# avlmaps/AVLMaps

Hardware: AMD Instinct MI355X
Metric: voxel_query_similarities_per_sec (higher is better)
Workload: dtype f32

## Files before the change

### avlmaps_amd/csrc/avl_sim.hip

```cpp
#include <cfloat>
#include <algorithm>
#include <climits>
#include <cstdlib>
#include <vector>

#include "avl_common.h"

namespace avl {

using half8 = __attribute__((ext_vector_type(8))) _Float16;
using half2 = __attribute__((ext_vector_type(2))) _Float16;
using f32x16 = __attribute__((ext_vector_type(16))) float;
using f32x4 = __attribute__((ext_vector_type(4))) float;

constexpr int kExactQB = 8;

template <bool VEC4>
__global__ __launch_bounds__(256) void sim_exact_kernel(const float* __restrict__ feat, int64_t N, int D, int64_t ld,
                                                        const float* __restrict__ q, int Q, int64_t ldq, int q0,
                                                        float* __restrict__ scores, int32_t* __restrict__ argmax,
                                                        float* __restrict__ best, int first_chunk) {
    extern __shared__ __attribute__((aligned(16))) float qs[];
    const int Dp = (D + 3) & ~3;
    const int qn = min(kExactQB, Q - q0);
// ... 46 lines not shown
            }
        }
#pragma unroll
        for (int r = 0; r < R; ++r)
#pragma unroll
            for (int j = 0; j < kExactQB; ++j) {
#pragma unroll
                for (int off = 32; off > 0; off >>= 1) acc[r][j] += __shfl_xor(acc[r][j], off, 64);
            }
#pragma unroll
        for (int r = 0; r < R; ++r) {
            const int64_t row = row0 + r;
            if (lane == r && row < N) {
                float bv = -INFINITY;
                int bi = q0;
                if (!first_chunk) {
                    if (best) bv = best[row];
                    if (argmax) bi = argmax[row];
                }
                bool have = !first_chunk;
#pragma unroll
                for (int j = 0; j < kExactQB; ++j) {
                    if (j < qn) {
                        if (scores) scores[row * (int64_t)Q + q0 + j] = acc[r][j];
                        if (!have || acc[r][j] > bv) {
                            bv = acc[r][j];
                            bi = q0 + j;
                            have = true;
                        }
                    }
                }
                if (argmax) argmax[row] = bi;
                if (best) best[row] = bv;
            }
        }
    }
}

constexpr int kHdrAlign = 256;
constexpr int kRowPadHalves = 8;
constexpr int kSplitThreads = 512;
#ifdef AVL_RING
template <bool PRE, bool XR, bool QM> struct RingDepth { static constexpr int value = AVL_RING; };
#else
#ifndef AVL_RING_QM
#define AVL_RING_QM 2
#endif
template <bool PRE, bool XR, bool QM> struct RingDepth { static constexpr int value = (!PRE && !XR) ? (QM ? AVL_RING_QM : 3) : 2; };
#endif
constexpr int kTileRows = (kSplitThreads / 64) * 32;

__global__ __launch_bounds__(256) void sim_prep_queries_kernel(const float* __restrict__ q, int Q, int D, int64_t ldq,
                                                               float* __restrict__ inv_scale, _Float16* __restrict__ img,
                                                               int Qtot, int KC, int nkc, int interleaved) {
    __shared__ float red[4];
    __shared__ float scale_s;
    const int qg = blockIdx.x;
    const bool live = qg < Q;
    const float* row = q + (int64_t)qg * ldq;
    float m = 0.f;
    if (live)
        for (int d = threadIdx.x; d < D; d += blockDim.x) m = fmaxf(m, fabsf(row[d]));
    for (int off = 32; off > 0; off >>= 1) m = fmaxf(m, __shfl_xor(m, off, 64));
    if ((threadIdx.x & 63) == 0) red[threadIdx.x >> 6] = m;
    __syncthreads();
    if (threadIdx.x == 0) {
        const float mx = fmaxf(fmaxf(red[0], red[1]), fmaxf(red[2], red[3]));
        int S = 0;
        if (mx > 0.f && isfinite(mx)) S = 9 - ilogbf(mx);
        S = max(-60, min(60, S));
        scale_s = ldexpf(1.f, S);
        inv_scale[qg] = ldexpf(1.f, -S);
    }
    __syncthreads();
    const float scale = scale_s;
    const int rowlen = KC + kRowPadHalves;
    if (interleaved) {
        const int rowblk = 2 * KC + kRowPadHalves;
        for (int kc = 0; kc < nkc; ++kc) {
            _Float16* hi = img + ((int64_t)kc * Qtot + qg) * rowblk;
            for (int kk = threadIdx.x; kk < KC + kRowPadHalves; kk += blockDim.x) {
                const int k = kc * KC + kk;
                float v = 0.f;
                if (live && kk < KC && k < D) v = row[k] * scale;
                const half2 h = __builtin_bit_cast(half2, __builtin_amdgcn_cvt_pkrtz(v, 0.f));
                if (kk < KC) {
                    hi[kk] = h[0];
                    hi[KC + kk] = (_Float16)(v - (float)h[0]);
                } else {
                    hi[KC + kk] = (_Float16)0;
                }
            }
        }
        return;
    }
    for (int kc = 0; kc < nkc; ++kc) {
        _Float16* hi = img + ((int64_t)(kc * 2) * Qtot + qg) * rowlen;
        _Float16* lo = hi + (int64_t)Qtot * rowlen;
        for (int kk = threadIdx.x; kk < rowlen; kk += blockDim.x) {
            const int k = kc * KC + kk;
            float v = 0.f;
            if (live && kk < KC && k < D) v = row[k] * scale;
            const half2 h = __builtin_bit_cast(half2, __builtin_amdgcn_cvt_pkrtz(v, 0.f));
            hi[kk] = h[0];
            lo[kk] = (_Float16)(v - (float)h[0]);
        }
    }
}

__device__ __forceinline__ void split8(const f32x4 v0, const f32x4 v1, half8& hi, half8& lo) {
#ifdef AVL_ABL_NOSPLIT
    hi = __builtin_bit_cast(half8, v0);
    lo = __builtin_bit_cast(half8, v1);
#else
    const float x[8] = {v0.x, v0.y, v0.z, v0.w, v1.x, v1.y, v1.z, v1.w};
    float m1 = -1.0f;
    asm("" : "+v"(m1));
#pragma unroll
    for (int p = 0; p < 4; ++p) {
        half2 h = __builtin_bit_cast(half2, __builtin_amdgcn_cvt_pkrtz(x[2 * p], x[2 * p + 1]));
        float r0 = __builtin_fmaf((float)h[0], m1, x[2 * p]);
        float r1 = __builtin_fmaf((float)h[1], m1, x[2 * p + 1]);
        half2 l = __builtin_bit_cast(half2, __builtin_amdgcn_cvt_pkrtz(r0, r1));
        hi[2 * p] = h[0];
        hi[2 * p + 1] = h[1];
        lo[2 * p] = l[0];
        lo[2 * p + 1] = l[1];
    }
#endif
}

constexpr float kGuardLo = 0x1p-7f, kGuardHi = 0x1p15f;

__device__ __forceinline__ void guard_max8(float& m, const f32x4 v0, const f32x4 v1) {
#ifndef AVL_GUARD_BUILTIN
    asm("v_max3_f32 %0, |%1|, |%2|, %0" : "+v"(m) : "v"(v0.x), "v"(v0.y));
    asm("v_max3_f32 %0, |%1|, |%2|, %0" : "+v"(m) : "v"(v0.z), "v"(v0.w));
    asm("v_max3_f32 %0, |%1|, |%2|, %0" : "+v"(m) : "v"(v1.x), "v"(v1.y));
    asm("v_max3_f32 %0, |%1|, |%2|, %0" : "+v"(m) : "v"(v1.z), "v"(v1.w));
#else
    m = __builtin_fmaxf(__builtin_fmaxf(m, __builtin_fabsf(v0.x)), __builtin_fabsf(v0.y));
    m = __builtin_fmaxf(__builtin_fmaxf(m, __builtin_fabsf(v0.z)), __builtin_fabsf(v0.w));
    m = __builtin_fmaxf(__builtin_fmaxf(m, __builtin_fabsf(v1.x)), __builtin_fabsf(v1.y));
    m = __builtin_fmaxf(__builtin_fmaxf(m, __builtin_fabsf(v1.z)), __builtin_fabsf(v1.w));
#endif
}

template <int QT, int NA, bool XR = false>
__device__ __forceinline__ void split_epilogue(const f32x16 (&acc)[QT][NA], const float* isc, int q_base, int rows, int Q,
                                               float* __restrict__ scores, int32_t* __restrict__ argmax,
                                               float* __restrict__ best, int64_t row, int64_t N, int kg, int first_chunk,
                                               float rscale = 1.f, uint32_t* __restrict__ flags = nullptr, float rmax = 1.f,
                                               const int32_t* qml = nullptr, f32x4 xacc = f32x4{0.f, 0.f, 0.f, 0.f}) {
    int lim = (XR ? 32 * QT : rows) - 4 * kg;
    asm volatile("" : "+v"(lim));
    float bv = -INFINITY;
    int bl = INT_MAX;
#pragma unroll
    for (int t = 0; t < QT; ++t) {
#pragma unroll
        for (int g = 0; g < 4; ++g) {
            const int c0 = t * 32 + 8 * g;
            const int ql = c0 + 4 * kg;
            const int qg = q_base + ql;
            const f32x4 is4 = *reinterpret_cast<const f32x4*>(isc + ql);
            f32x4 v;
            f32x4 r = {acc[t][0][4 * g + 0], acc[t][0][4 * g + 1], acc[t][0][4 * g + 2], acc[t][0][4 * g + 3]};
#pragma unroll
            for (int a = 1; a < NA; ++a) {
                r.x += acc[t][a][4 * g + 0]; r.y += acc[t][a][4 * g + 1]; r.z += acc[t][a][4 * g + 2]; r.w += acc[t][a][4 * g + 3];
            }
            v.x = r.x * is4.x * rscale;
            v.y = r.y * is4.y * rscale;
            v.z = r.z * is4.z * rscale;
            v.w = r.w * is4.w * rscale;
            if (scores && row < N) {
                float* sp = scores + row * (int64_t)Q + qg;
                if (qml) {
                    float* sr = scores + row * (int64_t)Q;
                    const int4 qm4 = *reinterpret_cast<const int4*>(qml + ql);
                    if (c0 + 0 < lim) sr[qm4.x] = v.x;
                    if (c0 + 1 < lim) sr[qm4.y] = v.y;
                    if (c0 + 2 < lim) sr[qm4.z] = v.z;
                    if (c0 + 3 < lim) sr[qm4.w] = v.w;
                } else if (c0 + 3 < lim && (Q & 3) == 0) {
                    *reinterpret_cast<f32x4*>(sp) = v;
                } else {
                    if (c0 + 0 < lim) sp[0] = v.x;
                    if (c0 + 1 < lim) sp[1] = v.y;
                    if (c0 + 2 < lim) sp[2] = v.z;
                    if (c0 + 3 < lim) sp[3] = v.w;
                }
            }
            if (c0 + 0 < lim && v.x > bv) { bv = v.x; bl = c0 + 0; }
            if (c0 + 1 < lim && v.y > bv) { bv = v.y; bl = c0 + 1; }
            if (c0 + 2 < lim && v.z > bv) { bv = v.z; bl = c0 + 2; }
            if (c0 + 3 < lim && v.w > bv) { bv = v.w; bl = c0 + 3; }
        }
    }
    int bi = bl == INT_MAX ? INT_MAX : q_base + 4 * kg + bl;
    float xv[4] = {0.f, 0.f, 0.f, 0.f};
    if constexpr (XR) {
        const f32x4 xis = *reinterpret_cast<const f32x4*>(isc + 32 * QT);
#pragma unroll
        for (int r = 0; r < 4; ++r) xv[r] = (xacc[r] + __shfl_xor(xacc[r], 32, 64)) * xis[r] * rscale;
        if (scores && row < N && kg == 0) {
            float* sr = scores + row * (int64_t)Q;
#pragma unroll
            for (int r = 0; r < 4; ++r)
                if (32 * QT + r < rows) sr[qml ? qml[32 * QT + r] : q_base + 32 * QT + r] = xv[r];
        }
    }
    if (argmax || best || flags) {
        if (qml && bi != INT_MAX) bi = qml[bi - q_base];
        const float ov = __shfl_xor(bv, 32, 64);
        const int oi = __shfl_xor(bi, 32, 64);
        if (ov > bv || (ov == bv && oi < bi)) {
            bv = ov;
            bi = oi;
        }
        if constexpr (XR) {
#pragma unroll
            for (int r = 0; r < 4; ++r)
                if (32 * QT + r < rows && xv[r] > bv) {
                    bv = xv[r];
                    bi = qml ? qml[32 * QT + r] : q_base + 32 * QT + r;
                }
        }
        if (flags) {
            const float m = fmaxf(rmax, __shfl_xor(rmax, 32, 64));
            const bool bad = row < N && (!(m == 0.f || (m >= kGuardLo && m < kGuardHi)) || bi == INT_MAX);
            const unsigned long long mask = __ballot(bad);
            const int64_t row0 = __shfl(row, 0, 64);
            if ((threadIdx.x & 63) == 0 && row0 < N) {
                const uint32_t w = (uint32_t)(mask | (mask >> 32));
                flags[row0 >> 5] = first_chunk ? w : (flags[row0 >> 5] | w);
            }
        }
        if ((argmax || best) && kg == 0 && row < N) {
            if (bi == INT_MAX) bi = qml ? qml[0] : q_base;
            if (!first_chunk) {
                const float pv = best[row];
                const int pi = argmax ? argmax[row] : -1;
                if (pv > bv || (pv == bv && pi < bi)) {
                    bv = pv;
                    bi = argmax ? pi : bi;
                }
            }
            if (argmax) argmax[row] = bi;
            if (best) best[row] = bv;
        }
    }
}

__global__ __launch_bounds__(256) void sim_prepare_map_kernel(float* __restrict__ feat, int64_t N, int D, int64_t ld,
                                                              float* __restrict__ row_scale) {
    const int lane = threadIdx.x & 63;
    const int64_t wave0 = ((int64_t)blockIdx.x * blockDim.x + threadIdx.x) >> 6;
    const int64_t nwaves = ((int64_t)gridDim.x * blockDim.x) >> 6;
    const int gpr = D >> 3;
    for (int64_t row = wave0; row < N; row += nwaves) {
        f32x4* p = reinterpret_cast<f32x4*>(feat + row * ld);
        float scale = 1.f;
        if (row_scale) {
            unsigned mb = 0;
            for (int g = lane; g < 2 * gpr; g += 64) {
                const f32x4 v = p[g];
                mb = max(max(mb, __float_as_uint(v.x) & 0x7fffffffu), __float_as_uint(v.y) & 0x7fffffffu);
                mb = max(max(mb, __float_as_uint(v.z) & 0x7fffffffu), __float_as_uint(v.w) & 0x7fffffffu);
            }
            for (int off = 32; off > 0; off >>= 1) mb = max(mb, (unsigned)__shfl_xor((int)mb, off, 64));
            int sh = 0;
            if (mb != 0 && mb < 0x7f800000u) sh = max(-100, min(100, 14 - ilogbf(__uint_as_float(mb))));
            scale = ldexpf(1.f, sh);
            if (lane == 0) row_scale[row] = mb >= 0x7f800000u ? __uint_as_float(0x7fc00000u) : ldexpf(1.f, -sh);
        }
        for (int g = lane; g < gpr; g += 64) {
            f32x4 v0 = p[2 * g], v1 = p[2 * g + 1];
            v0.x *= scale; v0.y *= scale; v0.z *= scale; v0.w *= scale;
            v1.x *= scale; v1.y *= scale; v1.z *= scale; v1.w *= scale;
            half8 hi, lo;
            split8(v0, v1, hi, lo);
            p[2 * g] = __builtin_bit_cast(f32x4, hi);
            p[2 * g + 1] = __builtin_bit_cast(f32x4, lo);
        }
    }
}

__host__ __device__ __forceinline__ int compact_lo_offset(int c) { return 128 * (c >> 7) + 64 * ((c >> 5) & 1) + 32 * ((c >> 6) & 1) + (c & 31); }

__global__ __launch_bounds__(256) void sim_prepare_map24_kernel(const float* __restrict__ feat, int64_t N, int D, int64_t ld,
                                                                unsigned char* __restrict__ out, float* __restrict__ row_scale) {
    const int lane = threadIdx.x & 63;
    const int64_t wave0 = ((int64_t)blockIdx.x * blockDim.x + threadIdx.x) >> 6;
    const int64_t nwaves = ((int64_t)gridDim.x * blockDim.x) >> 6;
    const int g8 = D >> 3;
    for (int64_t row = wave0; row < N; row += nwaves) {
        const f32x4* p = reinterpret_cast<const f32x4*>(feat + row * ld);
        unsigned mb = 0;
        for (int g = lane; g < 2 * g8; g += 64) {
            const f32x4 v = p[g];
            mb = max(max(mb, __float_as_uint(v.x) & 0x7fffffffu), __float_as_uint(v.y) & 0x7fffffffu);
            mb = max(max(mb, __float_as_uint(v.z) & 0x7fffffffu), __float_as_uint(v.w) & 0x7fffffffu);
        }
        for (int off = 32; off > 0; off >>= 1) mb = max(mb, (unsigned)__shfl_xor((int)mb, off, 64));
        int sh = 0;
        if (mb != 0 && mb < 0x7f800000u) sh = max(-100, min(100, 14 - ilogbf(__uint_as_float(mb))));
        const float scale = ldexpf(1.f, sh);
        if (lane == 0) row_scale[row] = mb >= 0x7f800000u ? __uint_as_float(0x7fc00000u) : ldexpf(1.f, -sh);
        unsigned char* orow = out + row * ((int64_t)D * 3);
        for (int g = lane; g < g8; g += 64) {
            const f32x4 v0 = p[2 * g], v1 = p[2 * g + 1];
            const float x[8] = {v0.x * scale, v0.y * scale, v0.z * scale, v0.w * scale, v1.x * scale, v1.y * scale, v1.z * scale, v1.w * scale};
            half8 hi;
            unsigned u[8];
#pragma unroll
            for (int e = 0; e < 8; ++e) {
                const _Float16 h = (_Float16)x[e];
                hi[e] = h;
                const int eb = (__builtin_bit_cast(unsigned short, h) >> 10) & 31;
                int k = 0;
#ifndef AVL_COMPACT_FIXED_UNITS
                if (eb > 18 && eb < 31) k = (int)rintf((x[e] - (float)h) * ldexpf(1.f, 33 - eb));
#else
                if (eb < 31) k = (int)rintf((x[e] - (float)h) * 16.f);
#endif
                u[e] = (unsigned)(max(-128, min(127, k)) + 128);
            }
            const int w0 = (int)(u[0] | (u[1] << 8) | (u[2] << 16) | (u[3] << 24));
            const int w1 = (int)(u[4] | (u[5] << 8) | (u[6] << 16) | (u[7] << 24));
            *reinterpret_cast<half8*>(orow + (size_t)g * 16) = hi;
            *reinterpret_cast<int2*>(orow + 2 * (size_t)D + compact_lo_offset(8 * g)) = int2{w0, w1};
        }
    }
}

__global__ __launch_bounds__(256) void sim_fixup_rows_kernel(const float* __restrict__ feat, int64_t N, int D, int64_t ld,
                                                             const float* __restrict__ q, int Q, int64_t ldq,
                                                             const uint32_t* __restrict__ flags, float* __restrict__ scores,
                                                             int32_t* __restrict__ argmax, float* __restrict__ best) {
    const int lane = threadIdx.x & 63;
    const int64_t wave0 = ((int64_t)blockIdx.x * blockDim.x + threadIdx.x) >> 6;
    const int64_t nwaves = ((int64_t)gridDim.x * blockDim.x) >> 6;
    const int64_t nwords = (N + 31) >> 5;
    for (int64_t base = wave0 * 64; base < nwords; base += nwaves * 64) {
        const uint32_t w = base + lane < nwords ? flags[base + lane] : 0u;
        unsigned long long any = __ballot(w != 0u);
        while (any) {
            const int l = __ffsll((long long)any) - 1;
            any &= any - 1;
            uint32_t word = (uint32_t)__shfl((int)w, l, 64);
            while (word) {
                const int b = __ffs((int)word) - 1;
                word &= word - 1;
                const int64_t row = (base + l) * 32 + b;
                if (row >= N) continue;
                const float* a = feat + row * ld;
                float bv = -INFINITY;
                int bi = 0;
                bool have = false, nan_seen = false;
                for (int qi = 0; qi < Q; ++qi) {
                    const float* qr = q + (int64_t)qi * ldq;
                    float sum = 0.f;
                    for (int d = lane; d < D; d += 64) sum = fmaf(a[d], qr[d], sum);
                    for (int off = 32; off > 0; off >>= 1) sum += __shfl_xor(sum, off, 64);
                    if (lane == 0 && scores) scores[row * (int64_t)Q + qi] = sum;
                    if (!nan_seen) {
                        if (sum != sum) { nan_seen = true; bv = sum; bi = qi; }
                        else if (!have || sum > bv) { bv = sum; bi = qi; have = true; }
                    }
                }
                if (lane == 0) {
                    if (argmax) argmax[row] = bi;
                    if (best) best[row] = bv;
                }
            }
        }
    }
}

__global__ __launch_bounds__(256) void sim_gather_queries_kernel(const float* __restrict__ q, int64_t ldq, const int32_t* __restrict__ rows,
                                                                 int nrows, int col0, int cols, float* __restrict__ out) {
    const int r = blockIdx.x;
    if (r >= nrows) return;
    const int32_t sr = rows[r];
    const float* src = q + (int64_t)(sr < 0 ? 0 : sr) * ldq + col0;
    float* dst = out + (int64_t)r * cols;
    for (int c = threadIdx.x; c < cols; c += blockDim.x) dst[c] = sr < 0 ? 0.f : src[c];
}


__device__ __forceinline__ void compact_load_step(f32x4 (&b)[8], const char* row, int64_t ld, int kg, int sa) {
    const f32x4* gh = reinterpret_cast<const f32x4*>(row + 128 * sa + 64 * kg);
    const f32x4* gl = reinterpret_cast<const f32x4*>(row + 2 * ld + 128 * (sa >> 1) + 64 * kg + 32 * (sa & 1));
#pragma unroll
    for (int t = 0; t < 4; ++t) b[t] = gh[t];
#pragma unroll
    for (int t = 0; t < 2; ++t) b[4 + t] = gl[t];
}

template <int PAIR>
__device__ __forceinline__ half2 residual_pair(unsigned w, unsigned hi2) {
#ifndef AVL_COMPACT_FIXED_UNITS
    using ushort2v = __attribute__((ext_vector_type(2))) unsigned short;
    const unsigned pat = __builtin_amdgcn_perm(0x64646464u, w, PAIR == 0 ? 0x04010400u : 0x04030402u);
    const half2 k = __builtin_bit_cast(half2, pat) + half2{(_Float16)-1152.0f, (_Float16)-1152.0f};
    const ushort2v e = __builtin_bit_cast(ushort2v, hi2 & 0x7C007C00u);
    const ushort2v sc = __builtin_elementwise_sub_sat(e, ushort2v{0x4800, 0x4800});
    return k * __builtin_bit_cast(half2, sc);
#else
    (void)hi2;
    const unsigned pat = __builtin_amdgcn_perm(0x54545454u, w, PAIR == 0 ? 0x04010400u : 0x04030402u);
    return __builtin_bit_cast(half2, pat) + half2{(_Float16)-72.0f, (_Float16)-72.0f};
#endif
}

__device__ __forceinline__ void compact_operands(const f32x4& hi, const f32x4& lo, int second, half8& bh, half8& bl) {
    bh = __builtin_bit_cast(half8, hi);
    using u32x4 = __attribute__((ext_vector_type(4))) unsigned;
    const u32x4 hw = __builtin_bit_cast(u32x4, hi);
    const u32x4 lw = __builtin_bit_cast(u32x4, lo);
    const unsigned w0 = lw[second * 2], w1 = lw[second * 2 + 1];
    const half2 l0 = residual_pair<0>(w0, hw[0]), l1 = residual_pair<1>(w0, hw[1]);
    const half2 l2 = residual_pair<0>(w1, hw[2]), l3 = residual_pair<1>(w1, hw[3]);
    bl = half8{l0[0], l0[1], l1[0], l1[1], l2[0], l2[1], l3[0], l3[1]};
}

template <bool PRE, bool P24>
__device__ __forceinline__ void map_operands(const f32x4 (&b)[8], int m, half8& bh, half8& bl, float& rmax) {
    if constexpr (P24) {
        compact_operands(b[m], b[4 + (m >> 1)], m & 1, bh, bl);
    } else if constexpr (PRE) {
        bh = __builtin_bit_cast(half8, b[2 * m]);
        bl = __builtin_bit_cast(half8, b[2 * m + 1]);
    } else {
#ifndef AVL_ABL_NOGUARD
        guard_max8(rmax, b[2 * m], b[2 * m + 1]);
#endif
        split8(b[2 * m], b[2 * m + 1], bh, bl);
    }
}

template <int QT, int NSTEPS, bool PRE, bool FQ, bool QM = false, bool P24 = false, bool XR = false>
__global__ __launch_bounds__(kSplitThreads) void sim_split_f16_kernel(
    const float* __restrict__ feat, int64_t N, int D, int64_t ld, const _Float16* __restrict__ img,
    const float* __restrict__ inv_scale, const float* __restrict__ q_raw, int64_t ldq, int Qtot, int KC, int nkc, int q_base,
    int rows, int Q, float* __restrict__ scores, int32_t* __restrict__ argmax, float* __restrict__ best, int first_chunk,
    const float* __restrict__ row_scale, uint32_t* __restrict__ flags, const int32_t* __restrict__ qmap, int col0) {
    extern __shared__ __attribute__((aligned(16))) char smem[];
    constexpr int NA = QT == 1 ? 3 : (QT == 2 ? 2 : 1);
    constexpr int X1 = NA > 1 ? 1 : 0, X2 = NA > 2 ? 2 : X1;
    const int lane = threadIdx.x & 63, wave = threadIdx.x >> 6;
    const int j = lane & 31, kg = lane >> 5;
    const int row_b = (KC + kRowPadHalves) * 2;
    static_assert(!XR || FQ, "the extra-row path builds its query image in the kernel");
    constexpr int TQ = (QT + (XR ? 1 : 0)) * 32;
    const int zrow = (FQ && rows < (XR ? 32 * QT + 4 : 32 * QT)) ? 1 : 0;
    const int img_b = (rows + zrow) * row_b;
    float* isc = reinterpret_cast<float*>(smem + 2 * img_b);
    int32_t* qml = reinterpret_cast<int32_t*>(isc + TQ);
    if constexpr (QM) {
        if (threadIdx.x < TQ) qml[threadIdx.x] = threadIdx.x < rows ? qmap[q_base + threadIdx.x] : INT_MAX;
    }
    if constexpr (!FQ) {
        if (threadIdx.x < TQ) isc[threadIdx.x] = threadIdx.x < rows ? inv_scale[q_base + threadIdx.x] : 0.f;
    } else {
        if (threadIdx.x >= rows && threadIdx.x < TQ) isc[threadIdx.x] = 0.f;
        constexpr int RB = 4, NW = kSplitThreads / 64;
        for (int r0 = wave; r0 < rows; r0 += NW * RB) {
            float v[RB][8];
#pragma unroll
            for (int b = 0; b < RB; ++b) {
                const int r = r0 + NW * b;
                const float* qr = q_raw + (int64_t)(q_base + (r < rows ? r : rows - 1)) * ldq;
#pragma unroll
                for (int t = 0; t < 8; ++t) v[b][t] = (lane + 64 * t < D) ? qr[lane + 64 * t] : 0.f;
            }
#pragma unroll
            for (int b = 0; b < RB; ++b) {
                const int r = r0 + NW * b;
                if (r < rows) {
                    float m = 0.f;
#pragma unroll
                    for (int t = 0; t < 8; ++t) m = fmaxf(m, fabsf(v[b][t]));
                    for (int off = 32; off > 0; off >>= 1) m = fmaxf(m, __shfl_xor(m, off, 64));
                    int S = 0;
                    if (m > 0.f && isfinite(m)) S = 9 - ilogbf(m);
                    S = max(-60, min(60, S));
                    const float scale = ldexpf(1.f, S);
                    if (lane == 0) isc[r] = ldexpf(1.f, -S);
                    _Float16* hi = reinterpret_cast<_Float16*>(smem + r * row_b);
                    _Float16* lo = reinterpret_cast<_Float16*>(smem + img_b + r * row_b);
#pragma unroll
                    for (int t = 0; t < 8; ++t) {
                        const int k = lane + 64 * t;
                        if (k < KC) {
                            const float x = v[b][t] * scale;
                            const half2 h = __builtin_bit_cast(half2, __builtin_amdgcn_cvt_pkrtz(x, 0.f));
                            hi[k] = h[0];
                            lo[k] = (_Float16)(x - (float)h[0]);
                        }
                    }
                    if (lane < kRowPadHalves) {
                        hi[KC + lane] = (_Float16)0;
                        lo[KC + lane] = (_Float16)0;
                    }
                }
            }
        }
        if (zrow) {
            uint32_t* zh = reinterpret_cast<uint32_t*>(smem + rows * row_b);
            uint32_t* zl = reinterpret_cast<uint32_t*>(smem + img_b + rows * row_b);
            for (int i = threadIdx.x; i < row_b / 4; i += kSplitThreads) {
                zh[i] = 0u;
                zl[i] = 0u;
            }
        }
    }

    auto fill_lds = [&](int kc) {
        const char* hi = reinterpret_cast<const char*>(img) + ((int64_t)(kc * 2) * Qtot + q_base) * row_b;
        const char* lo = hi + (int64_t)Qtot * row_b;
        const uint4* s0 = reinterpret_cast<const uint4*>(hi);
        const uint4* s1 = reinterpret_cast<const uint4*>(lo);
        uint4* d0 = reinterpret_cast<uint4*>(smem);
        uint4* d1 = reinterpret_cast<uint4*>(smem + img_b);
        for (int i = threadIdx.x; i < img_b / 16; i += kSplitThreads) {
// ... 123 lines not shown
                f32x4 hb[2][4], lb[2][4];
                auto load_hi = [&](int st) {
                    const f32x4* g = reinterpret_cast<const f32x4*>(rp24 + 128 * (sa0 + st) + 64 * kg);
#pragma unroll
                    for (int t = 0; t < 4; ++t) hb[st & 1][t] = g[t];
                };
                auto load_lo = [&](int blk) {
                    const f32x4* g = reinterpret_cast<const f32x4*>(rp24 + 2 * ld + 128 * ((sa0 >> 1) + blk) + 64 * kg);
#pragma unroll
                    for (int t = 0; t < 4; ++t) lb[blk & 1][t] = g[t];
                };
                load_hi(0);
                load_lo(0);
#pragma unroll
                for (int st = 0; st < NSTEPS; ++st) {
                    if (st + 1 < NSTEPS) {
                        load_hi(st + 1);
                        if (((st + 1) & 1) == 0) load_lo((st + 1) >> 1);
                    }
                    __builtin_amdgcn_sched_barrier(0);
                    compute_with([&](int m, half8& bh, half8& bl) {
                        compact_operands(hb[st & 1][m], lb[(st >> 1) & 1][2 * (st & 1) + (m >> 1)], m & 1, bh, bl);
                    }, st);
                }
            } else if constexpr (NSTEPS > 0) {
                constexpr int kRing = RingDepth<PRE, XR, QM>::value;
                f32x4 ring[kRing][8];
#pragma unroll
                for (int r = 0; r + 1 < kRing; ++r)
                    if (r < NSTEPS) load(ring[r], r);
#pragma unroll
                for (int s = 0; s < NSTEPS; ++s) {
                    if (s + kRing - 1 < NSTEPS) load(ring[(s + kRing - 1) % kRing], s + kRing - 1);
                    __builtin_amdgcn_sched_barrier(0);
                    compute(ring[s % kRing], s);
                }
            } else {
                load(buf0, 0);
                for (int s = 0; s < nsteps; s += 2) {
                    if (s + 1 < nsteps) load(buf1, s + 1);
                    compute(buf0, s);
                    if (s + 1 < nsteps) {
                        if (s + 2 < nsteps) load(buf0, s + 2);
                        compute(buf1, s + 1);
                    }
                }
            }
        }

        float rscale = 1.f;
        if constexpr (PRE) {
            if (row_scale) rscale = row_scale[rowc];
        }
        split_epilogue<QT, NA, XR>(acc, isc, q_base, rows, Q, scores, argmax, best, row, N, kg, first_chunk, rscale, PRE ? nullptr : flags, rmax,
                                   QM ? qml : nullptr, xacc0 + xacc1);
    }
}

template <int QT, int T, int NS, bool PRE, bool QM = false, bool P24 = false>
__global__ __launch_bounds__(kSplitThreads) void sim_kswap_f16_kernel(
    const float* __restrict__ feat, int64_t N, int D, int64_t ld, const _Float16* __restrict__ img,
    const float* __restrict__ inv_scale, int Qtot, int KC, int q_base, int rows, int Q, float* __restrict__ scores,
    int32_t* __restrict__ argmax, float* __restrict__ best, int first_chunk, const float* __restrict__ row_scale,
    uint32_t* __restrict__ flags, const int32_t* __restrict__ qmap, int col0) {
    extern __shared__ __attribute__((aligned(16))) char smem[];
    const int lane = threadIdx.x & 63, wave = threadIdx.x >> 6;
    const int j = lane & 31, kg = lane >> 5;
    const int row_b = (KC + kRowPadHalves) * 2;
    const int zrow = rows < 32 * QT ? 1 : 0;
    const int img_b = (rows + zrow) * row_b;
    float* isc = reinterpret_cast<float*>(smem + 2 * img_b);
    int32_t* qml = reinterpret_cast<int32_t*>(isc + QT * 32);
    if constexpr (QM) {
        if (threadIdx.x < QT * 32) qml[threadIdx.x] = threadIdx.x < rows ? qmap[q_base + threadIdx.x] : INT_MAX;
    }
    if (threadIdx.x < QT * 32) isc[threadIdx.x] = threadIdx.x < rows ? inv_scale[q_base + threadIdx.x] : 0.f;
    auto fill_lds = [&](int kc) {
        using gptr = const __attribute__((address_space(1))) void*;
        using lptr = __attribute__((address_space(3))) void*;
        const char* hi = reinterpret_cast<const char*>(img) + ((int64_t)(kc * 2) * Qtot + q_base) * row_b;
        const char* lo = hi + (int64_t)Qtot * row_b;
        const int nb = rows * row_b;
        for (int c = wave * 1024; c < nb; c += (kSplitThreads / 64) * 1024) {
            if (c + lane * 16 < nb) {
                __builtin_amdgcn_global_load_lds((gptr)(hi + c + lane * 16), (lptr)(smem + c), 16, 0, 0);
                __builtin_amdgcn_global_load_lds((gptr)(lo + c + lane * 16), (lptr)(smem + img_b + c), 16, 0, 0);
            }
        }
    };
    auto fill_wait = [&]() { asm volatile("s_waitcnt vmcnt(0)" ::: "memory"); };
    if (zrow)
        for (int i = threadIdx.x; i < row_b / 4; i += kSplitThreads) {
            reinterpret_cast<uint32_t*>(smem + rows * row_b)[i] = 0u;
            reinterpret_cast<uint32_t*>(smem + img_b + rows * row_b)[i] = 0u;
        }
    fill_lds(0);
    fill_wait();
    __syncthreads();

    const char* a_base[QT];
#pragma unroll
    for (int t = 0; t < QT; ++t) a_base[t] = smem + min(t * 32 + j, rows - 1 + zrow) * row_b + kg * 64;

    const int64_t G = gridDim.x;
    const int64_t R = N / (G * kTileRows);
    const int64_t tail_row0 = R * G * kTileRows;
    const int64_t tail_units = (N - tail_row0 + 31) / 32;
    const int64_t tu0 = tail_units * blockIdx.x / G, tu1 = tail_units * (blockIdx.x + 1) / G;
// ... 831 lines not shown
    if (QT == 2) return reinterpret_cast<const void*>(sim_kswap_f16_kernel<2, AVL_KSWAP_T, NS, PRE, QM, P24>);
    return reinterpret_cast<const void*>(sim_kswap_f16_kernel<1, 2 * AVL_KSWAP_T, 0, PRE, QM, P24>);
}
template <bool PRE, bool QM, bool P24>
static const void* pick_kswap_kernel(int QT, int ns) {
    return ns == 8 ? pick_kswap_kernel_ns<8, PRE, QM, P24>(QT) : (ns == 6 ? pick_kswap_kernel_ns<6, PRE, QM, P24>(QT) : pick_kswap_kernel_ns<0, PRE, QM, P24>(QT));
}

static bool split_plan_is_fused(const SplitPlan& p, int D) { return !p.stream && p.nkc == 1 && D <= 512; }

template <int QT, bool QM>
static const void* pick_split24_kernel(bool s8, bool fq) {
    if (fq) return s8 ? reinterpret_cast<const void*>(sim_split_f16_kernel<QT, 8, true, true, QM, true>)
                      : reinterpret_cast<const void*>(sim_split_f16_kernel<QT, 0, true, true, QM, true>);
    return reinterpret_cast<const void*>(sim_split_f16_kernel<QT, 0, true, false, QM, true>);
}

template <int QT>
static const void* pick_split_xr_kernel(bool prepared, bool p24) {
    if (p24) return reinterpret_cast<const void*>(sim_split_f16_kernel<QT, 8, true, true, false, true, true>);
    if (prepared) return reinterpret_cast<const void*>(sim_split_f16_kernel<QT, 8, true, true, false, false, true>);
    return reinterpret_cast<const void*>(sim_split_f16_kernel<QT, 8, false, true, false, false, true>);
}

template <int QT, bool PRE, bool QM>
static const void* pick_split_kernel(bool s8, bool fq) {
    if (fq) return s8 ? reinterpret_cast<const void*>(sim_split_f16_kernel<QT, 8, PRE, true, QM>)
                      : reinterpret_cast<const void*>(sim_split_f16_kernel<QT, 0, PRE, true, QM>);
    return reinterpret_cast<const void*>(sim_split_f16_kernel<QT, 0, PRE, false, QM>);
}

static int run_fixup(const float* d_feat, int64_t N, int D, int64_t ld, const float* d_q, int Q, int64_t ldq, const uint32_t* d_flags,
                     float* d_scores, int32_t* d_argmax, float* d_best, hipStream_t st) {
    const int64_t nwords = (N + 31) >> 5;
    int64_t blocks = (nwords + 255) / 256;
    const int64_t maxb = (int64_t)num_cus() * 8;
    if (blocks > maxb) blocks = maxb;
    if (blocks < 1) blocks = 1;
    hipLaunchKernelGGL(sim_fixup_rows_kernel, dim3((unsigned)blocks), dim3(256), 0, st, d_feat, N, D, ld, d_q, Q, ldq, d_flags, d_scores,
                       d_argmax, d_best);
    AVL_HIP_CHECK(hipGetLastError());
    return AVL_OK;
}

template <bool PRE>
static int run_split(const float* d_feat, int64_t N, int D, int64_t ld, const float* d_q, int Qg, int64_t ldq, int Qs,
                     float* d_scores, int32_t* d_argmax, float* d_best, const SplitPlan& p, void* d_ws, const float* d_row_scale,
                     uint32_t* d_flags, const int32_t* d_qmap, bool first_launch, hipStream_t st, bool p24 = false, int col0 = 0) {
    float* inv_scale = reinterpret_cast<float*>(d_ws);
    _Float16* img = reinterpret_cast<_Float16*>(reinterpret_cast<char*>(d_ws) + p.hdr_bytes);
    const bool fq = split_plan_is_fused(p, D);
    if (!fq)
        hipLaunchKernelGGL(sim_prep_queries_kernel, dim3(p.Qtot), dim3(256), 0, st, d_q, Qg, D, ldq, inv_scale, img, p.Qtot, p.KC,
                           p.nkc, p.stream ? 1 : 0);
    const int64_t ntiles = (N + kTileRows - 1) / kTileRows;
    int64_t blocks = ntiles < num_cus() ? ntiles : num_cus();
    if (blocks < 1) blocks = 1;
    if (p.stream) {
        for (int ci = 0; ci < p.nchunks; ++ci) {
            const SplitChunk& c = p.chunks[ci];
            const bool tb = ((ld * (p24 ? 3 : 4)) % 4096) != 0;
            const void* kern = nullptr;
            if constexpr (PRE) {
                if (p24) kern = d_qmap ? pick_stream_kernel_spc<true, true, true>(p.SPC, c.QT, tb) : pick_stream_kernel_spc<true, false, true>(p.SPC, c.QT, tb);
            }
            if (!kern) kern = d_qmap ? pick_stream_kernel_spc<PRE, true, false>(p.SPC, c.QT, tb) : pick_stream_kernel_spc<PRE, false, false>(p.SPC, c.QT, tb);
            const size_t lds = p.lds_bytes(c);
            int rc = ensure_dynamic_lds(kern, lds);
            if (rc != AVL_OK) return rc;
            const _Float16* img_c = img;
            const float* isc_c = inv_scale;
            int Qtot = p.Qtot, nch = p.nkc, q_base = c.q_base, rows = c.rows, first = (ci == 0 && first_launch) ? 1 : 0;
            void* args[] = {&d_feat, &N, &D, &ld, &img_c, &isc_c, &Qtot, &nch, &q_base, &rows, &Qs, &d_scores, &d_argmax, &d_best, &first,
                            &d_row_scale, &d_flags, &d_qmap, &col0};
            AVL_HIP_CHECK(hipLaunchKernel(kern, dim3((unsigned)blocks), dim3(kSplitThreads), args, lds, st));
        }
        AVL_HIP_CHECK(hipGetLastError());
        return AVL_OK;
    }
    if (p.kswap) {
        const SplitChunk& c = p.chunks[0];
        const int s8 = (p24 && col0 % 128 != 0) ? 0 : ((p.KC == 512 && D == 1024) ? 8 : ((p.KC == 384 && D == 768) ? 6 : 0));
        const void* kern = nullptr;
        if constexpr (PRE) {
            if (p24) kern = d_qmap ? pick_kswap_kernel<true, true, true>(c.QT, s8) : pick_kswap_kernel<true, false, true>(c.QT, s8);
        }
        if (!kern) kern = d_qmap ? pick_kswap_kernel<PRE, true, false>(c.QT, s8) : pick_kswap_kernel<PRE, false, false>(c.QT, s8);
        const size_t lds = p.lds_bytes(c);
        int rc = ensure_dynamic_lds(kern, lds);
        if (rc != AVL_OK) return rc;
        const _Float16* img_c = img;
        const float* isc_c = inv_scale;
        int Qtot = p.Qtot, KC = p.KC, q_base = c.q_base, rows = c.rows, first = first_launch ? 1 : 0;
        void* args[] = {&d_feat, &N, &D, &ld, &img_c, &isc_c, &Qtot, &KC, &q_base, &rows, &Qs, &d_scores, &d_argmax, &d_best, &first,
                        &d_row_scale, &d_flags, &d_qmap, &col0};
        AVL_HIP_CHECK(hipLaunchKernel(kern, dim3((unsigned)blocks), dim3(kSplitThreads), args, lds, st));
        AVL_HIP_CHECK(hipGetLastError());
        return AVL_OK;
    }
    for (int ci = 0; ci < p.nchunks; ++ci) {
        const SplitChunk& c = p.chunks[ci];
        const bool s8 = (p.nkc == 1 && D == 512) && (!p24 || col0 % 128 == 0);
        const int xr = c.rows % 32;
        const bool use_xr = kSimExtraRows && s8 && fq && !d_qmap && xr >= 1 && xr <= 4 && c.rows > 32 && c.rows / 32 <= 2 &&
                            (PRE || c.rows / 32 == 2);
        const void* kern = use_xr ? (c.rows / 32 == 2 ? pick_split_xr_kernel<2>(PRE, p24) : pick_split_xr_kernel<1>(PRE, p24))
                           : (p24 && d_qmap) ? (c.QT == 3 ? pick_split24_kernel<3, true>(s8, fq) : (c.QT == 2 ? pick_split24_kernel<2, true>(s8, fq) : pick_split24_kernel<1, true>(s8, fq)))
// ... 118 lines not shown
    if (precision == AVL_SIM_EXACT_VALU) use_split = false;
    else if (precision == AVL_SIM_EXACT) {
        use_split = false;
        use_f32_mfma = can_split;
    } else if (precision == AVL_SIM_SPLIT_F16 || precision == AVL_SIM_PREPARED) {
        AVL_REQUIRE(can_split, "avl_sim_scores: SPLIT_F16 needs D %% 64 == 0 and 16-byte aligned rows (D=%d ld=%lld)", D,
                    (long long)ld_feat);
        use_split = true;
    } else use_split = can_split;

    std::vector<ColGroup> groups;
    std::vector<SplitPlan> gplans;
    if (use_split && h_col_begin && h_col_end) {
        make_col_groups(D, Q, h_col_begin, h_col_end, groups);
        bool ok = groups.size() > 1 && groups.size() <= 16;
        for (size_t g = 0; ok && g < groups.size(); ++g) {
            SplitPlan gp;
            ok = make_split_plan(groups[g].cols, (int)groups[g].rows.size(), gp, true);
            gplans.push_back(gp);
        }
        if (!ok) { groups.clear(); gplans.clear(); }
    }
    const bool blocks = !groups.empty();

    float* best = d_best;
    int32_t* amax = d_argmax;
    float* tmp_best = nullptr;
    int32_t* tmp_amax = nullptr;
    int nlaunch = (use_split || use_f32_mfma) ? p.nchunks : (Q + kExactQB - 1) / kExactQB;
    if (blocks) {
        nlaunch = 0;
        for (const SplitPlan& gp : gplans) nlaunch += gp.nchunks;
    }
    if (nlaunch > 1 && (d_argmax || d_best)) {
        if (!best) {
            AVL_HIP_CHECK(hipMallocAsync(reinterpret_cast<void**>(&tmp_best), (size_t)N * sizeof(float), st));
            best = tmp_best;
        }
        if (!amax && blocks) {
            AVL_HIP_CHECK(hipMallocAsync(reinterpret_cast<void**>(&tmp_amax), (size_t)N * sizeof(int32_t), st));
            amax = tmp_amax;
        }
    }
    int rc = AVL_OK;
    if (use_split || use_f32_mfma) {
        const bool prepared = precision == AVL_SIM_PREPARED;
        size_t img_bytes = 0;
        if (blocks) {
            for (const SplitPlan& gp : gplans) img_bytes = img_bytes > gp.ws_bytes ? img_bytes : gp.ws_bytes;
        } else if (use_f32_mfma || !split_plan_is_fused(p, D)) {
            img_bytes = p.ws_bytes;
        }
        img_bytes = img_bytes ? align_up(img_bytes, kHdrAlign) : 0;
        const size_t flag_bytes = (use_split && !prepared) ? guard_bytes(N) : 0;
        const size_t blk_bytes = blocks ? blocks_bytes(D, Q) : 0;
        const size_t need = img_bytes + flag_bytes + blk_bytes;
        char* ws = static_cast<char*>(d_workspace);
        void* tmp_ws = nullptr;
        if (need > 0 && (!ws || workspace_bytes < need)) {
            AVL_HIP_CHECK(hipMallocAsync(&tmp_ws, need, st));
            ws = static_cast<char*>(tmp_ws);
        }
        uint32_t* flags = flag_bytes ? reinterpret_cast<uint32_t*>(ws + img_bytes) : nullptr;
        if (!use_split) {
            rc = run_mfma_f32(d_feat, N, D, ld_feat, d_queries, Q, ld_q, d_scores, amax, best, p, ws, st);
        } else if (!blocks) {
            rc = prepared ? run_split<true>(d_feat, N, D, ld_feat, d_queries, Q, ld_q, Q, d_scores, amax, best, p, ws, d_row_scale, nullptr,
                                            nullptr, true, st, p24)
                          : run_split<false>(d_feat, N, D, ld_feat, d_queries, Q, ld_q, Q, d_scores, amax, best, p, ws, nullptr, flags,
                                             nullptr, true, st);
        } else {
            float* qg = reinterpret_cast<float*>(ws + img_bytes + flag_bytes);
            int32_t* qmap = reinterpret_cast<int32_t*>(ws + img_bytes + flag_bytes + align_up((size_t)Q * D * sizeof(float), kHdrAlign));
            std::vector<int32_t> h_map;
            h_map.reserve((size_t)Q);
            for (const ColGroup& g : groups) h_map.insert(h_map.end(), g.rows.begin(), g.rows.end());
            AVL_HIP_CHECK(hipMemcpyAsync(qmap, h_map.data(), (size_t)Q * sizeof(int32_t), hipMemcpyHostToDevice, st));
            size_t row_off = 0, qg_off = 0;
            for (size_t g = 0; g < groups.size() && rc == AVL_OK; ++g) {
                const ColGroup& cg = groups[g];
                const int Qg = (int)cg.rows.size();
                float* qg_g = qg + qg_off;
                const int32_t* qmap_g = qmap + row_off;
                hipLaunchKernelGGL(sim_gather_queries_kernel, dim3((unsigned)Qg), dim3(256), 0, st, d_queries, ld_q, qmap_g, Qg, cg.col0,
                                   cg.cols, qg_g);
                const float* feat_g = p24 ? d_feat : d_feat + cg.col0;
                rc = prepared ? run_split<true>(feat_g, N, cg.cols, ld_feat, qg_g, Qg, cg.cols, Q, d_scores, amax, best, gplans[g], ws,
                                                d_row_scale, nullptr, qmap_g, g == 0, st, p24, p24 ? cg.col0 : 0)
                              : run_split<false>(feat_g, N, cg.cols, ld_feat, qg_g, Qg, cg.cols, Q, d_scores, amax, best, gplans[g], ws, nullptr,
                                                 flags, qmap_g, g == 0, st);
                row_off += (size_t)Qg;
                qg_off += (size_t)Qg * cg.cols;
            }
        }
        if (rc == AVL_OK && use_split && !prepared)
            rc = run_fixup(d_feat, N, D, ld_feat, d_queries, Q, ld_q, flags, d_scores, d_argmax, d_best, st);
        if (tmp_ws) (void)hipFreeAsync(tmp_ws, st);
    } else {
        rc = run_exact(d_feat, N, D, ld_feat, d_queries, Q, ld_q, d_scores, d_argmax, best, st);
    }
    if (tmp_best) (void)hipFreeAsync(tmp_best, st);
    if (tmp_amax) (void)hipFreeAsync(tmp_amax, st);
    return rc;
}

int avl_sim_scores_ws(const float* d_feat, int64_t N, int D, int64_t ld_feat, const float* d_queries, int Q,
                      int64_t ld_q, float* d_scores, int32_t* d_argmax, float* d_best, int precision,
                      void* d_workspace, size_t workspace_bytes, void* stream) {
    return sim_scores_impl(d_feat, nullptr, N, D, ld_feat, d_queries, Q, ld_q, d_scores, d_argmax, d_best, precision, d_workspace,
                           workspace_bytes, stream);
}

int avl_sim_scores_blocks(const float* d_feat, const float* d_row_scale, int64_t N, int D, int64_t ld_feat, const float* d_queries,
                          int Q, int64_t ld_q, const int32_t* h_col_begin, const int32_t* h_col_end, float* d_scores,
                          int32_t* d_argmax, float* d_best, int precision, void* d_workspace, size_t workspace_bytes, void* stream) {
    AVL_REQUIRE(h_col_begin && h_col_end, "avl_sim_scores_blocks: null column support");
    return sim_scores_impl(d_feat, d_row_scale, N, D, ld_feat, d_queries, Q, ld_q, d_scores, d_argmax, d_best, precision, d_workspace,
                           workspace_bytes, stream, h_col_begin, h_col_end);
}

int avl_sim_scores_prepared(const float* d_feat, const float* d_row_scale, int64_t N, int D, int64_t ld_feat,
                            const float* d_queries, int Q, int64_t ld_q, float* d_scores, int32_t* d_argmax, float* d_best,
                            void* d_workspace, size_t workspace_bytes, void* stream) {
    return sim_scores_impl(d_feat, d_row_scale, N, D, ld_feat, d_queries, Q, ld_q, d_scores, d_argmax, d_best, AVL_SIM_PREPARED,
                           d_workspace, workspace_bytes, stream);
}

int avl_sim_scores_prepared24(const void* d_map24, const float* d_row_scale, int64_t N, int D, const float* d_queries, int Q,
                              int64_t ld_q, float* d_scores, int32_t* d_argmax, float* d_best, void* d_workspace,
                              size_t workspace_bytes, void* stream) {
    AVL_REQUIRE(d_row_scale, "avl_sim_scores_prepared24: the compact form always has row scales");
    return sim_scores_impl(reinterpret_cast<const float*>(d_map24), d_row_scale, N, D, D, d_queries, Q, ld_q, d_scores, d_argmax, d_best,
                           AVL_SIM_PREPARED24, d_workspace, workspace_bytes, stream);
}

int avl_sim_prepare_map24(const float* d_feat, int64_t N, int D, int64_t ld_feat, void* d_map24, float* d_row_scale, void* stream) {
    AVL_REQUIRE(N >= 0 && D > 0 && ld_feat >= D, "avl_sim_prepare_map24: bad shape");
    AVL_REQUIRE(D % 128 == 0 && ld_feat % 4 == 0 && (reinterpret_cast<uintptr_t>(d_feat) & 15) == 0 &&
                    (reinterpret_cast<uintptr_t>(d_map24) & 15) == 0,
                "avl_sim_prepare_map24: needs D %% 128 == 0 (whole 128-column residual lines) and 16-byte aligned rows (D=%d ld=%lld)", D,
                (long long)ld_feat);
    if (N == 0) return AVL_OK;
    AVL_REQUIRE(d_feat && d_map24 && d_row_scale, "avl_sim_prepare_map24: null pointer");
    int64_t blocks = (N + 3) / 4;
    const int64_t maxb = (int64_t)num_cus() * 16;
    if (blocks > maxb) blocks = maxb;
    hipLaunchKernelGGL(sim_prepare_map24_kernel, dim3((unsigned)blocks), dim3(256), 0, as_stream(stream), d_feat, N, D, ld_feat,
                       reinterpret_cast<unsigned char*>(d_map24), d_row_scale);
// ... 112 lines not shown
```

Measured before the change: 179.2 billion.

## Inline guard fixup into split epilogue and drop query gather kernel

When the split path is fused and single-chunk, the exact-recompute fixup for rows that fail the fp16 range guard now runs inside the epilogue of the main kernel. This removes the separate fixup launch and the flag buffer. The block path also stops gathering queries into a scratch buffer; it reads the original query rows through the qmap indirection in the prep and fused-load code. This saves launches and a copy, but adds divergent slow-path code and extra register pressure to the hot epilogue.

```diff
diff --git a/avlmaps_amd/csrc/avl_sim.hip b/avlmaps_amd/csrc/avl_sim.hip
--- a/avlmaps_amd/csrc/avl_sim.hip
+++ b/avlmaps_amd/csrc/avl_sim.hip
@@ -122,12 +122,13 @@
 
 __global__ __launch_bounds__(256) void sim_prep_queries_kernel(const float* __restrict__ q, int Q, int D, int64_t ldq,
                                                                float* __restrict__ inv_scale, _Float16* __restrict__ img,
-                                                               int Qtot, int KC, int nkc, int interleaved) {
+                                                               int Qtot, int KC, int nkc, int interleaved,
+                                                               const int32_t* __restrict__ qmap) {
     __shared__ float red[4];
     __shared__ float scale_s;
     const int qg = blockIdx.x;
     const bool live = qg < Q;
-    const float* row = q + (int64_t)qg * ldq;
+    const float* row = q + (int64_t)(live && qmap ? qmap[qg] : qg) * ldq;
     float m = 0.f;
     if (live)
         for (int d = threadIdx.x; d < D; d += blockDim.x) m = fmaxf(m, fabsf(row[d]));
@@ -216,12 +217,45 @@
 #endif
 }
 
-template <int QT, int NA, bool XR = false>
+__device__ __forceinline__ void fixup_row(const float* __restrict__ feat, int D, int64_t ld, const float* __restrict__ q, int Q,
+                                          int64_t ldq, int64_t row, int lane, float* __restrict__ scores,
+                                          int32_t* __restrict__ argmax, float* __restrict__ best) {
+    const float* a = feat + row * ld;
+    float bv = -INFINITY;
+    int bi = 0;
+    bool have = false, nan_seen = false;
+    for (int qi = 0; qi < Q; ++qi) {
+        const float* qr = q + (int64_t)qi * ldq;
+        float sum = 0.f;
+        for (int d = lane; d < D; d += 64) sum = fmaf(a[d], qr[d], sum);
+        for (int off = 32; off > 0; off >>= 1) sum += __shfl_xor(sum, off, 64);
+        if (lane == 0 && scores) scores[row * (int64_t)Q + qi] = sum;
+        if (!nan_seen) {
+            if (sum != sum) { nan_seen = true; bv = sum; bi = qi; }
+            else if (!have || sum > bv) { bv = sum; bi = qi; have = true; }
+        }
+    }
+    if (lane == 0) {
+        if (argmax) argmax[row] = bi;
+        if (best) best[row] = bv;
+    }
+}
+
+struct FixupArgs {
+    const float* feat;
+    int D;
+    int64_t ld;
+    const float* q;
+    int64_t ldq;
+};
+
+template <int QT, int NA, bool XR = false, bool INL = false>
 __device__ __forceinline__ void split_epilogue(const f32x16 (&acc)[QT][NA], const float* isc, int q_base, int rows, int Q,
                                                float* __restrict__ scores, int32_t* __restrict__ argmax,
                                                float* __restrict__ best, int64_t row, int64_t N, int kg, int first_chunk,
                                                float rscale = 1.f, uint32_t* __restrict__ flags = nullptr, float rmax = 1.f,
-                                               const int32_t* qml = nullptr, f32x4 xacc = f32x4{0.f, 0.f, 0.f, 0.f}) {
+                                               const int32_t* qml = nullptr, f32x4 xacc = f32x4{0.f, 0.f, 0.f, 0.f},
+                                               const FixupArgs& fx = FixupArgs{}) {
     int lim = (XR ? 32 * QT : rows) - 4 * kg;
     asm volatile("" : "+v"(lim));
     float bv = -INFINITY;
@@ -281,7 +315,7 @@
                 if (32 * QT + r < rows) sr[qml ? qml[32 * QT + r] : q_base + 32 * QT + r] = xv[r];
         }
     }
-    if (argmax || best || flags) {
+    if (argmax || best || flags || INL) {
         if (qml && bi != INT_MAX) bi = qml[bi - q_base];
         const float ov = __shfl_xor(bv, 32, 64);
         const int oi = __shfl_xor(bi, 32, 64);
@@ -297,14 +331,18 @@
                     bi = qml ? qml[32 * QT + r] : q_base + 32 * QT + r;
                 }
         }
-        if (flags) {
+        unsigned long long mask = 0ull;
+        if (flags || INL) {
             const float m = fmaxf(rmax, __shfl_xor(rmax, 32, 64));
             const bool bad = row < N && (!(m == 0.f || (m >= kGuardLo && m < kGuardHi)) || bi == INT_MAX);
-            const unsigned long long mask = __ballot(bad);
-            const int64_t row0 = __shfl(row, 0, 64);
-            if ((threadIdx.x & 63) == 0 && row0 < N) {
-                const uint32_t w = (uint32_t)(mask | (mask >> 32));
-                flags[row0 >> 5] = first_chunk ? w : (flags[row0 >> 5] | w);
+            mask = __ballot(bad);
+            if (flags) {
+                const int64_t row0 = __shfl(row, 0, 64);
+                if ((threadIdx.x & 63) == 0 && row0 < N) {
+                    const uint32_t w = (uint32_t)(mask | (mask >> 32));
+                    flags[row0 >> 5] = first_chunk ? w : (flags[row0 >> 5] | w);
+                }
+                mask = 0ull;
             }
         }
         if ((argmax || best) && kg == 0 && row < N) {
@@ -319,6 +357,19 @@
             }
             if (argmax) argmax[row] = bi;
             if (best) best[row] = bv;
+        }
+        if constexpr (INL) {
+            uint32_t word = (uint32_t)(mask | (mask >> 32));
+            if (word) {
+                __builtin_amdgcn_fence(__ATOMIC_SEQ_CST, "agent");
+                int lane = threadIdx.x & 63;
+                asm volatile("" : "+v"(lane));
+                while (word) {
+                    const int b = __ffs((int)word) - 1;
+                    word &= word - 1;
+                    fixup_row(fx.feat, fx.D, fx.ld, fx.q, Q, fx.ldq, __shfl(row, b, 64), lane, scores, argmax, best);
+                }
+            }
         }
     }
 }
@@ -425,38 +476,10 @@
                 word &= word - 1;
                 const int64_t row = (base + l) * 32 + b;
                 if (row >= N) continue;
-                const float* a = feat + row * ld;
-                float bv = -INFINITY;
-                int bi = 0;
-                bool have = false, nan_seen = false;
-                for (int qi = 0; qi < Q; ++qi) {
-                    const float* qr = q + (int64_t)qi * ldq;
-                    float sum = 0.f;
-                    for (int d = lane; d < D; d += 64) sum = fmaf(a[d], qr[d], sum);
-                    for (int off = 32; off > 0; off >>= 1) sum += __shfl_xor(sum, off, 64);
-                    if (lane == 0 && scores) scores[row * (int64_t)Q + qi] = sum;
-                    if (!nan_seen) {
-                        if (sum != sum) { nan_seen = true; bv = sum; bi = qi; }
-                        else if (!have || sum > bv) { bv = sum; bi = qi; have = true; }
-                    }
-                }
-                if (lane == 0) {
-                    if (argmax) argmax[row] = bi;
-                    if (best) best[row] = bv;
-                }
-            }
-        }
-    }
-}
-
-__global__ __launch_bounds__(256) void sim_gather_queries_kernel(const float* __restrict__ q, int64_t ldq, const int32_t* __restrict__ rows,
-                                                                 int nrows, int col0, int cols, float* __restrict__ out) {
-    const int r = blockIdx.x;
-    if (r >= nrows) return;
-    const int32_t sr = rows[r];
-    const float* src = q + (int64_t)(sr < 0 ? 0 : sr) * ldq + col0;
-    float* dst = out + (int64_t)r * cols;
-    for (int c = threadIdx.x; c < cols; c += blockDim.x) dst[c] = sr < 0 ? 0.f : src[c];
+                fixup_row(feat, D, ld, q, Q, ldq, row, lane, scores, argmax, best);
+            }
+        }
+    }
 }
 
 
@@ -542,7 +565,8 @@
 #pragma unroll
             for (int b = 0; b < RB; ++b) {
                 const int r = r0 + NW * b;
-                const float* qr = q_raw + (int64_t)(q_base + (r < rows ? r : rows - 1)) * ldq;
+                const int qrow = q_base + (r < rows ? r : rows - 1);
+                const float* qr = q_raw + (int64_t)(QM ? qmap[qrow] : qrow) * ldq;
 #pragma unroll
                 for (int t = 0; t < 8; ++t) v[b][t] = (lane + 64 * t < D) ? qr[lane + 64 * t] : 0.f;
             }
@@ -772,8 +796,9 @@
         if constexpr (PRE) {
             if (row_scale) rscale = row_scale[rowc];
         }
-        split_epilogue<QT, NA, XR>(acc, isc, q_base, rows, Q, scores, argmax, best, row, N, kg, first_chunk, rscale, PRE ? nullptr : flags, rmax,
-                                   QM ? qml : nullptr, xacc0 + xacc1);
+        constexpr bool INL = !PRE && FQ && !QM;
+        split_epilogue<QT, NA, XR, INL>(acc, isc, q_base, rows, Q, scores, argmax, best, row, N, kg, first_chunk, rscale, PRE ? nullptr : flags,
+                                        rmax, QM ? qml : nullptr, xacc0 + xacc1, FixupArgs{feat, D, ld, q_raw, ldq});
     }
 }
 
@@ -1711,7 +1736,7 @@
     const bool fq = split_plan_is_fused(p, D);
     if (!fq)
         hipLaunchKernelGGL(sim_prep_queries_kernel, dim3(p.Qtot), dim3(256), 0, st, d_q, Qg, D, ldq, inv_scale, img, p.Qtot, p.KC,
-                           p.nkc, p.stream ? 1 : 0);
+                           p.nkc, p.stream ? 1 : 0, d_qmap);
     const int64_t ntiles = (N + kTileRows - 1) / kTileRows;
     int64_t blocks = ntiles < num_cus() ? ntiles : num_cus();
     if (blocks < 1) blocks = 1;
@@ -1936,8 +1961,9 @@
             img_bytes = p.ws_bytes;
         }
         img_bytes = img_bytes ? align_up(img_bytes, kHdrAlign) : 0;
-        const size_t flag_bytes = (use_split && !prepared) ? guard_bytes(N) : 0;
-        const size_t blk_bytes = blocks ? blocks_bytes(D, Q) : 0;
+        const bool one_launch = use_split && !prepared && !blocks && split_plan_is_fused(p, D) && p.nchunks == 1;
+        const size_t flag_bytes = (use_split && !prepared && !one_launch) ? guard_bytes(N) : 0;
+        const size_t blk_bytes = blocks ? align_up((size_t)Q * sizeof(int32_t), kHdrAlign) : 0;
         const size_t need = img_bytes + flag_bytes + blk_bytes;
         char* ws = static_cast<char*>(d_workspace);
         void* tmp_ws = nullptr;
@@ -1954,30 +1980,26 @@
                           : run_split<false>(d_feat, N, D, ld_feat, d_queries, Q, ld_q, Q, d_scores, amax, best, p, ws, nullptr, flags,
                                              nullptr, true, st);
         } else {
-            float* qg = reinterpret_cast<float*>(ws + img_bytes + flag_bytes);
-            int32_t* qmap = reinterpret_cast<int32_t*>(ws + img_bytes + flag_bytes + align_up((size_t)Q * D * sizeof(float), kHdrAlign));
+            int32_t* qmap = reinterpret_cast<int32_t*>(ws + img_bytes + flag_bytes);
             std::vector<int32_t> h_map;
             h_map.reserve((size_t)Q);
             for (const ColGroup& g : groups) h_map.insert(h_map.end(), g.rows.begin(), g.rows.end());
             AVL_HIP_CHECK(hipMemcpyAsync(qmap, h_map.data(), (size_t)Q * sizeof(int32_t), hipMemcpyHostToDevice, st));
-            size_t row_off = 0, qg_off = 0;
+            size_t row_off = 0;
             for (size_t g = 0; g < groups.size() && rc == AVL_OK; ++g) {
                 const ColGroup& cg = groups[g];
                 const int Qg = (int)cg.rows.size();
-                float* qg_g = qg + qg_off;
                 const int32_t* qmap_g = qmap + row_off;
-                hipLaunchKernelGGL(sim_gather_queries_kernel, dim3((unsigned)Qg), dim3(256), 0, st, d_queries, ld_q, qmap_g, Qg, cg.col0,
-                                   cg.cols, qg_g);
                 const float* feat_g = p24 ? d_feat : d_feat + cg.col0;
-                rc = prepared ? run_split<true>(feat_g, N, cg.cols, ld_feat, qg_g, Qg, cg.cols, Q, d_scores, amax, best, gplans[g], ws,
+                const float* q_g = d_queries + cg.col0;
+                rc = prepared ? run_split<true>(feat_g, N, cg.cols, ld_feat, q_g, Qg, ld_q, Q, d_scores, amax, best, gplans[g], ws,
                                                 d_row_scale, nullptr, qmap_g, g == 0, st, p24, p24 ? cg.col0 : 0)
-                              : run_split<false>(feat_g, N, cg.cols, ld_feat, qg_g, Qg, cg.cols, Q, d_scores, amax, best, gplans[g], ws, nullptr,
+                              : run_split<false>(feat_g, N, cg.cols, ld_feat, q_g, Qg, ld_q, Q, d_scores, amax, best, gplans[g], ws, nullptr,
                                                  flags, qmap_g, g == 0, st);
                 row_off += (size_t)Qg;
-                qg_off += (size_t)Qg * cg.cols;
-            }
-        }
-        if (rc == AVL_OK && use_split && !prepared)
+            }
+        }
+        if (rc == AVL_OK && use_split && !prepared && !one_launch)
             rc = run_fixup(d_feat, N, D, ld_feat, d_queries, Q, ld_q, flags, d_scores, d_argmax, d_best, st);
         if (tmp_ws) (void)hipFreeAsync(tmp_ws, st);
     } else {
```

Result: faster. 182.2 billion, median of 6 (+1.6%).
